# nguyenduchuyiu/marl-delivery

Hardware: AMD Instinct MI355X
Metric: agent-steps/sec (whole node), map1 5-agent 4096 envs, 1/2/4/8 MI355X (higher is better)
Workload: dtype int32+fp64

## Files before the change

### marl-delivery_amd/csrc/mdl_step_halves.hpp

```cpp
#pragma once

constexpr int HALF = 32;
constexpr int HALF_NC = 4;
constexpr int HALVES_MAX_P = HALF * HALF_NC;
constexpr int HALF_CAND = 136;

__device__ __forceinline__ uint32_t half_min_u32(uint32_t m) {
    m = row_min_u32(m);
    const auto r = __builtin_amdgcn_permlane16_swap(m, m, false, false);
    return r[0] < r[1] ? r[0] : r[1];
}

constexpr size_t HALF_GREC = (size_t)HALF_NC * 64 * 8, HALF_GPS = (size_t)HALF_NC * 64 * 2;
__host__ __device__ constexpr size_t halves_scratch_bytes() {
    return HALF_GREC + HALF_GPS + 64 * (size_t)HALF_NC + 2 * (size_t)HALF_CAND * 8;
}

struct HalvesLayout {
    static constexpr int G = HALF, NC = HALF_NC;
    static constexpr uint32_t ROFF_MASK = 0x1fu;
    static constexpr uint32_t RESET_OFF_MASK = 0xffu;
    static constexpr size_t FLAG_OFF = HALF_GREC + HALF_GPS;
    static constexpr bool RANK_BEFORE_RESET = false;
    __device__ static __forceinline__ bool stores_robot(const GroupLane q) { return (q.lane & 16) == 0; }

    struct Near {
        int stc[NC];
        uint64_t anyw;
        uint64_t* cand;
        int nwg;
    };
    template <bool STALE>
    __device__ static __forceinline__ void near_pre(Near& nr, const GroupLane q, unsigned char* slice,
                                                    const uint32_t (&ps0)[NC], const uint64_t (&td)[NC], int t0, bool, int) {
        uint64_t wvm[NC];
        bool wv[NC];
        nr.anyw = 0;
#pragma unroll
        for (int c = 0; c < NC; c++) {
            wv[c] = !(MDL_ABLATE & 64) && trk_waiting<STALE>(ps0[c], td[c], t0);
            nr.stc[c] = pk_start(td[c]);
            wvm[c] = ballot(wv[c]);
            nr.anyw |= wvm[c];
        }
        nr.cand = (uint64_t*)(slice + HALF_GREC + HALF_GPS + 64 * NC) + q.g * HALF_CAND;
        nr.nwg = 0;
        if (nr.anyw) {
            int n0 = 0, n1 = 0;
#pragma unroll
            for (int c = 0; c < NC; c++) {
                const int lo = popc64(wvm[c] & 0x00000000ffffffffull);
                const int below = (int)__builtin_amdgcn_mbcnt_hi((uint32_t)(wvm[c] >> 32),
                                                                 __builtin_amdgcn_mbcnt_lo((uint32_t)wvm[c], 0u));
                const int idx = below + (q.g ? n1 - lo : n0);
                const uint32_t j = (uint32_t)(c * HALF + q.gl);
                const uint32_t klo = (near_order<STALE, HALF * NC>(ps0[c], j) << 7) | j;
                if (wv[c]) nr.cand[idx] = (uint64_t)(uint32_t)nr.stc[c] | ((uint64_t)klo << 32);
                n0 += lo;
                n1 += popc64(wvm[c] & 0xffffffff00000000ull);
            }
            const int nh = q.g ? n1 : n0;
            nr.nwg = (max(n0, n1) + 3) & ~3;
            for (int k = nh + q.gl; k < nr.nwg; k += HALF) nr.cand[k] = 0x0000ffffffffffffull;
        }
    }
    __device__ static __forceinline__ void near_post(const Near& nr, const GroupLane q, bool, bool act, int pcell, int cell,
                                                     uint32_t& Midle, uint32_t& Mcan, int& best_cell) {
        if (nr.anyw && !(MDL_ABLATE & 32)) {
            const uint64_t* cp = nr.cand + ((q.lane >> 4) & 1);
            uint32_t kmin = 0xffffffffu;
            uint64_t hmc = 0;
            for (int i0 = 0; i0 < nr.nwg; i0 += 4) {
                const uint64_t ce = cp[i0], cf = cp[i0 + 2];
                const uint32_t ke = __builtin_amdgcn_sad_hi_u8((uint32_t)pcell, (uint32_t)ce, (uint32_t)(ce >> 32));
                const uint32_t kf = __builtin_amdgcn_sad_hi_u8((uint32_t)pcell, (uint32_t)cf, (uint32_t)(cf >> 32));
                kmin = min(kmin, min(ke, kf));
                hmc |= ballot((int)(uint32_t)ce == cell) | ballot((int)(uint32_t)cf == cell);
            }
            {
                const auto r = __builtin_amdgcn_permlane16_swap(kmin, kmin, false, false);
                kmin = r[0] < r[1] ? r[0] : r[1];
            }
            const uint32_t h16 = (uint32_t)(((hmc >> q.gbase) | (hmc >> (q.gbase + 16))) & 0xffffull);
            Mcan = ((h16 >> q.ri) & 1u) ? ~0u : 0u;
            const int js = (int)(kmin & 127u);
            const int sl = (q.gbase + (js & 31)) << 2;
            int bc = __builtin_amdgcn_ds_bpermute(sl, nr.stc[0]);
#pragma unroll
            for (int c = 1; c < NC; c++) {
                const int v = __builtin_amdgcn_ds_bpermute(sl, nr.stc[c]);
                bc = (js >> 5) == c ? v : bc;
            }
            const bool found = act && kmin < (509u << 16);
            Midle = lmask(found && (kmin >> 16) <= 3u);
            best_cell = found ? bc : -1;
        }
    }

    __device__ static __forceinline__ void gather_put(unsigned char* slice, int lane, const uint32_t (&ps0)[NC],
                                                      const uint64_t (&pk)[NC], const uint64_t (&td)[NC]) {
        uint64_t* grec = (uint64_t*)slice;
        uint16_t* gps = (uint16_t*)(slice + HALF_GREC);
#pragma unroll
        for (int c = 0; c < NC; c++) {
            grec[c * 64 + lane] = (uint64_t)tgt_dl(pk[c]) | ((uint64_t)tgt_dl(td[c]) << 32);
            gps[c * 64 + lane] = (uint16_t)ps0[c];
        }
    }
    __device__ static __forceinline__ void gather_get(unsigned char* slice, const GroupLane q, int pj, uint32_t& g_pf,
                                                      uint32_t& g_pk, uint32_t& g_td) {
        const int gi = ((pj >> 5) & (NC - 1)) * 64 + q.gbase + (pj & 31);
        const uint64_t gv = ((const uint64_t*)slice)[gi];
        g_pf = ((const uint16_t*)(slice + HALF_GREC))[gi], g_pk = (uint32_t)gv, g_td = (uint32_t)(gv >> 32);
    }

    __device__ static __forceinline__ void partners(const GroupLane q, bool act, bool mover, uint64_t, int prop, int cell,
                                                    bool& blocked, int& occ) {
        const uint32_t wd = (mover ? (uint32_t)prop : 0xffffu) | ((act ? (uint32_t)cell : 0xfffeu) << 16);
        const int g8 = (q.lane & 16) >> 1;
        uint32_t hk = 0;
        int ok = -1;
#pragma unroll
        for (int k = 0; k < 8; k++) {
            const uint32_t wj = (uint32_t)__builtin_amdgcn_ds_bpermute((q.gbase + g8 + k) << 2, (int)wd);
            hk |= (wj & 0xffffu) == (uint32_t)prop ? (1u << k) : 0u;
            ok = (wj >> 16) == (uint32_t)prop ? k : ok;
        }
        uint32_t hit = hk << g8;
        occ = ok < 0 ? -1 : ok + g8;
        {
            const auto rh = __builtin_amdgcn_permlane16_swap(hit, hit, false, false);
            hit = rh[0] | rh[1];
            const auto ro = __builtin_amdgcn_permlane16_swap((uint32_t)occ, (uint32_t)occ, false, false);
            occ = max((int)ro[0], (int)ro[1]);
        }
        blocked = (hit & ((1u << q.ri) - 1u)) != 0u;
    }

    __device__ static __forceinline__ void pickups(const GroupLane q, unsigned char* slice, uint32_t nw, bool picker,
                                                   uint64_t pickers, const int (&sw)[NC], int cell, int& cnew) {
        constexpr uint32_t NONE = 255u;
        if (nw & NW_SMALLMAP) {
            uint32_t* pb = (uint32_t*)slice + q.g * 128;
            auto word_of = [](int cl) { return (((uint32_t)cl >> 7) | (((uint32_t)cl >> 5) & 1u)) & 127u; };
            wave_sync();
            reinterpret_cast<u32x4*>((uint32_t*)slice)[q.lane] = u32x4{0u, 0u, 0u, 0u};
            wave_sync();
            if (picker && stores_robot(q)) atomicOr(&pb[word_of(cell)], 1u << (cell & 31));
            wave_sync();
            uint64_t left = pickers & 0x0000ffff0000ffffull;
#pragma unroll
            for (int c = 0; c < NC; c++) {
                const uint32_t bit = __builtin_amdgcn_ubfe(pb[word_of(sw[c])], (uint32_t)sw[c] & 31u, 1u);
                const uint64_t mt = ballot((sw[c] >= 0) & (bit != 0u));
                for (uint64_t m = mt; m && left; m &= m - 1) {
                    const int j = ffs64(m);
                    const uint64_t who = ballot(cell == rdl(sw[c], j)) & left & (0xffffull << (j & 32));
                    if (who) {
                        const int i = ffs64(who);
                        left &= ~(1ull << i);
                        cnew = (q.lane & ~16) == i ? c * HALF + (j & 31) + 1 : cnew;
                    }
                }
            }
        } else
        for (uint32_t u = rows_union(pickers); u; u &= u - 1) {
            const int J = __ffs((int)u) - 1;
            const int ci = __builtin_amdgcn_ds_bpermute((q.rbase + J) << 2, cell);
            uint32_t k = NONE;
#pragma unroll
            for (int c = NC - 1; c >= 0; c--) k = sw[c] == ci ? (uint32_t)(c * HALF + q.gl) : k;
            k = half_min_u32(k);
            cnew = (q.ri == J && picker && k != NONE) ? (int)k + 1 : cnew;
        }
    }

    __device__ static __forceinline__ float agent_sum(float s_lane, int) {
        const float r8 = s_lane + dppf<0x128>(s_lane);
        const float s2 = r8 + dppf<0xB1>(r8);
        const float c4 = s2 + dppf<0x4E>(s2);
        const float d = c4 + dppf<0x124>(c4);
        return 0.0f + row_bcastf<0>(d);
    }

    __device__ static __forceinline__ ResetLds reset_robots(uint32_t (&)[NC], unsigned char* slice, const GroupLane q,
                                                            const DevParams& p, int P, uint32_t, int er2, int gb, int mi,
                                                            int mvoff, bool store, GLOBAL uint32_t* robe) {
        ResetLds L = reset_carve(slice, P);
        const int mr = rdl(mi, gb);
        const MapDesc md = p.maps[mr];
        const int nc = do_reset(p, er2, md, L, false);
        const int ncr = __builtin_amdgcn_ds_bpermute(q.ri << 2, nc);
        if (store) *robe = rob_pack(ncr, 0, p.movevalid_cell[(uint32_t)(mvoff + ncr)]);
        return L;
    }
};
```

### marl-delivery_amd/csrc/mdl_step_multi.hpp

```cpp
#pragma once

struct GroupLane {
    int lane;
    int g, gl, gbase;
    int rbase, ri;
};
template <bool STALE, int MAXP>
__device__ __forceinline__ uint32_t near_order(uint32_t f, uint32_t j) {
    return STALE ? ((f & PS_SURVIVOR) ? (f >> PS_RANK_SHIFT) : (uint32_t)MAXP + j) : j;
}

#include "mdl_step_rows.hpp"
#include "mdl_step_halves.hpp"

template <bool STALE, int G, int NC>
__device__ __forceinline__ void rank_survivors(uint32_t (&ps)[NC], const GroupLane q, int P, int gb, bool mine) {
    constexpr uint64_t GMASK = ~0ull >> (64 - G);
    uint32_t rk[NC], tq[NC];
#pragma unroll
    for (int c = 0; c < NC; c++) {
        rk[c] = 0;
        tq[c] = order_key<STALE>(ps[c], c * G + q.gl);
    }
#pragma unroll
    for (int c2 = 0; c2 < NC; c2++) {
        uint64_t pm = ballot(c2 * G + q.gl < P && (ps[c2] & PS_PRESENT)) & (GMASK << gb);
        while (pm) {
            const uint32_t ki = (uint32_t)rdl((int)tq[c2], ffs64(pm));
            pm &= pm - 1;
#pragma unroll
            for (int c = 0; c < NC; c++) rk[c] += ki < tq[c] ? 1u : 0u;
        }
    }
#pragma unroll
    for (int c = 0; c < NC; c++) {
        if (mine) {
            if (c * G + q.gl < P && (ps[c] & PS_PRESENT)) {
                ps[c] = (ps[c] & PS_FLAGS) | PS_SURVIVOR | (rk[c] << PS_RANK_SHIFT);
            } else {
                ps[c] &= PS_STATUS;
            }
        }
    }
}

template <class L, bool STALE, int NFULL>
__device__ __forceinline__ void step_groups(const uint32_t* __restrict__ rob_pre, const uint64_t* __restrict__ pkg_pre,
                                            const uint16_t* __restrict__ pst_pre, const u32x4* __restrict__ es_pre,
                                            const uint64_t* __restrict__ trk_pre, const uint8_t* __restrict__ act_pre,
                                            uint32_t ap, uint32_t nw, const StepArgs& args) {
    constexpr int G = L::G, LG = G == 16 ? 4 : 5, NC = L::NC, NG = WAVE / G, MAX_P = G * NC;
    static_assert(G == 1 << LG, "groups of 16 or 32 lanes");
    constexpr uint64_t GMASK = ~0ull >> (64 - G);
    static_assert(NC == 4, "one flag byte per package slot, a lane's NC slots in one 32-bit load");
    constexpr int MAX_OFF = (NG - 1) * MAX_P + (G - 1) + (NC - 1) * G;
    static_assert(MAX_OFF < PKG_PAD && MAX_OFF <= 0xff, "step_groups: package loads stay inside the buffers' padding");
    extern __shared__ __align__(16) unsigned char smem[];
    const DevParams& p = args.p;
    const StepPre pre(rob_pre, pkg_pre, pst_pre, es_pre, trk_pre, act_pre, ap, nw);
    const int A = pre.A, P = pre.P;

    const int wave = wave_id();
    const int lane = lane_id();
    const int w = pre.slot() * pre.wpb + wave;
    const int e0 = NG * w;
    if (wave >= pre.wpb || e0 >= pre.n) return;
    const GroupLane q{lane, lane >> LG, lane & (G - 1), lane & (WAVE - G), lane & 48, lane & 15};
    const bool live = e0 + q.g < pre.n;
    const int ge = live ? q.g : 0;
    const bool act = live && q.ri < A;
    const bool rstore = L::stores_robot(q);

    const uint32_t roff = (uint32_t)(q.g * A + q.ri);
    const uint32_t roff_c = (act ? roff : 0u) & L::ROFF_MASK;
    const uint32_t rv_ld = (pre.rob + (size_t)e0 * A)[roff_c];
    const uint32_t ar_ld = (pre.act + (size_t)e0 * A)[roff_c];
    uint64_t pk[NC], td[NC];
    uint32_t ps[NC], ps_in[NC];
    bool dirty[NC];
    GLOBAL const uint64_t* pkge = pre.pkg + (size_t)e0 * P;
    GLOBAL const uint16_t* pste = pre.pst + (size_t)e0 * P;
    GLOBAL const uint64_t* trke = pre.trk + (size_t)e0 * P;
    bool pv[NC];
    const uint32_t lb = (uint32_t)(ge * P + q.gl) & 0xffu;
#pragma unroll
    for (int c = 0; c < NC; c++) {
        pv[c] = c < NFULL || c * G + q.gl < P;
        pk[c] = pkge[lb + c * G];
        ps[c] = pste[lb + c * G];
        td[c] = STALE ? trke[lb + c * G] : 0ull;
        dirty[c] = false;
    }
    const uint32_t erow = (uint32_t)ge & (NG - 1);
    const uint32_t t_ld = ((GLOBAL const uint32_t*)(pre.es + e0))[4u * erow];
    const uint64_t tot_ld = ((GLOBAL const uint64_t*)(pre.es + e0))[2u * erow + 1u];
    KargPtr kap = (KargPtr)((__attribute__((address_space(4))) const char*)__builtin_amdgcn_kernarg_segment_ptr() +
                            offsetof(StepKarg, args));
    const double cst = kap->p.cost_fold[q.gl];
    __builtin_amdgcn_sched_barrier(0);
    const uint32_t rv = act ? rv_ld : 0u;
    int araw = act ? (int)(ar_ld & 0xffu) : 0;
    const uint32_t t_rec = t_ld;
    const uint64_t tot_rec = tot_ld;
#pragma unroll
    for (int c = 0; c < NC; c++) {
        if (c >= NFULL) {
            pk[c] = pv[c] ? pk[c] : ~0ull;
            ps[c] = pv[c] ? ps[c] : (uint32_t)ST_DELIVERED;
            td[c] = pv[c] ? td[c] : ~0ull;
        }
        ps_in[c] = ps[c];
    }
    const int fmt = args.fmt, auto_reset = args.auto_reset, lds_stride = args.lds_stride;
    const int T = p.T;
    unsigned char* slice = smem + (size_t)wave * lds_stride;
    int mvoff = p.maps[0].mvc_off;
    int mi = 0;
    if (nw & NW_MAP) {
        mi = (int)((GLOBAL const uint8_t*)p.env_map)[e0 + ge];
#pragma unroll
        for (int k = 1; k < MAX_MAPS; k++) mvoff = (mi == k) ? p.maps[k].mvc_off : mvoff;
    }
    int cell = rob_cell(rv), carry = rob_carry(rv);
    uint32_t vmask = rob_valid(rv);
    const int t0 = (int)t_rec;
    const double tot_cur = __hiloint2double((int)(uint32_t)(tot_rec >> 32), (int)(uint32_t)tot_rec);

    int mv, op;
    decode_action(araw, fmt, mv, op);
    mv = act ? mv : MV_S;
    op = act ? op : 0;
    uint32_t ps0[NC];
#pragma unroll
    for (int c = 0; c < NC; c++) {
        ps0[c] = ps[c];
        if (!STALE || !(ps0[c] & PS_SURVIVOR)) td[c] = pk[c];
    }

    typename L::Near nr;
    L::template near_pre<STALE>(nr, q, slice, ps0, td, t0, act, cell);

    const int pj = carry - 1;
    unsigned char* flb = slice + L::FLAG_OFF;
    L::gather_put(slice, lane, ps0, pk, td);
    ((uint32_t*)flb)[lane] = 0;
    wave_sync();
    uint32_t g_pf, g_pk, g_td;
    L::gather_get(slice, q, pj, g_pf, g_pk, g_td);

    const int pcell = cell, pcarry = carry;
    const int prop = move_proposal(act, cell, vmask, mv);
    const bool mover = !(MDL_ABLATE & 4) && act && prop != cell;
    const uint64_t movers = ballot(mover);
    const uint32_t pvm = (uint32_t)(p.movevalid_cell + mvoff)[(uint32_t)prop];
    uint64_t moved = 0;
    if (movers) {
        bool blocked;
        int occ;
        L::partners(q, act, mover, movers, prop, cell, blocked, occ);
        const uint32_t Mbase = lmask(mover && !blocked), Mfree = lmask(occ < 0);
        moved = ballot((Mbase & Mfree) != 0u);
        if (ballot((Mbase & ~Mfree) != 0u)) {
            const int oln = q.rbase + (occ & 15);
            for (int it = 0; it < A; it++) {
                const uint64_t nm = ballot((Mbase & (Mfree | vbit(moved, oln))) != 0u);
                if (nm == moved) break;
                moved = nm;
            }
        }
        if ((moved >> lane) & 1ull) cell = prop;
    }
    const int n_cost = (int)__popc(row_bits(moved, q.rbase));

    const bool picker = !(MDL_ABLATE & 8) && act && op == 1 && carry == 0;
    const uint64_t pickers = ballot(picker);
    int cnew = carry;
    if (pickers) {
        int sw[NC];
#pragma unroll
        for (int c = 0; c < NC; c++) sw[c] = (ps[c] & PS_STATUS) == ST_WAITING ? pk_start(pk[c]) : -2;
        L::pickups(q, slice, nw, picker, pickers, sw, cell, cnew);
    }
    const bool picked = cnew != carry;
    carry = cnew;
    const int g_tgt = (int)(g_pk & 0xffffu), g_dl = (int)(g_pk >> 16);
    const bool drop = act && op == 2 && carry != 0 && g_tgt == cell;
    const uint64_t dmask = ballot(drop), omask = ballot(drop && t0 <= g_dl);
    constexpr uint32_t F_CHG = 8u, F_CARRY = 4u;
    {
        const int fs = drop ? pj : carry - 1;
        const uint32_t fv = picked ? (F_CHG | F_CARRY | (uint32_t)ST_IN_TRANSIT)
                            : drop ? (F_CHG | (uint32_t)ST_DELIVERED) : F_CARRY;
        if (act && rstore && carry != 0) flb[(q.gbase + (fs & (G - 1))) * NC + (fs >> LG)] = (unsigned char)fv;
    }
    carry = drop ? 0 : carry;
    wave_sync();
    const uint32_t fw = ((const uint32_t*)flb)[lane];
#pragma unroll
    for (int c = 0; c < NC; c++) {
        const uint32_t f = fw >> (8 * c);
        const uint32_t clr = (0u - ((f >> 3) & 1u)) & PS_STATUS;
        ps[c] = (ps[c] & ~clr) | (f & PS_STATUS);
    }
    double rr;
    {
        const int src = (q.gbase + n_cost) << 2;
        const uint32_t lo = (uint32_t)__builtin_amdgcn_ds_bpermute(src, (int)__double2loint(cst));
        const uint32_t hi = (uint32_t)__builtin_amdgcn_ds_bpermute(src, (int)__double2hiint(cst));
        rr = __hiloint2double((int)hi, (int)lo);
    }
    const uint32_t drow = row_bits(dmask, q.rbase), orow = row_bits(omask, q.rbase);
    if (dmask) {
        double DR = p.delivery_reward, DL = p.delay_reward;
        pin(DR);
        pin(DL);
        for (uint32_t u = rows_union(dmask); u; u &= u - 1) {
            const int i = __ffs((int)u) - 1;
            const double add = ((orow >> i) & 1u) ? DR : DL;
            rr = ((drow >> i) & 1u) ? rr + add : rr;
        }
    }
    const uint32_t rfl = (n_cost ? RT_MOVE : 0u) | (orow ? RT_ONTIME : 0u) | ((drow & ~orow) ? RT_LATE : 0u);
    const int t1 = t0 + 1;
    const double total = tot_cur + rr;

    uint32_t undel = 0;
    uint64_t spawned = 0;
#pragma unroll
    for (int c = 0; c < NC; c++) {
        undel |= (ps[c] & PS_STATUS) ^ (uint32_t)ST_DELIVERED;
        const bool sp = pk_st(pk[c]) == t1;
        spawned |= ballot(sp);
        ps[c] = sp ? ((ps[c] & ~PS_STATUS) | ST_WAITING) : ps[c];
    }
    const uint32_t alldel = lmask(((ballot(undel != 0u) >> q.gbase) & GMASK) == 0ull);
    const bool done = (lmask(live) & (lmask(t1 == T) | alldel)) != 0u;

    float s_lane;
    {
        const ShapeMasks<STALE> M(act, pcarry, carry, P, g_pf, pcell, cell, mv, op);
        uint32_t Midle = 0, Mcan = 0;
        int best_cell = -1;
        L::near_post(nr, q, M.need_can(), act, pcell, cell, Midle, Mcan, best_cell);
        const ShapeConsts C(p);
        s_lane = shape_terms<STALE>(M, C, (int)(g_td & 0xffffu), (int)(g_td >> 16), t1, best_cell, Midle, Mcan, pcell, cell);
    }
    const float shaped = (float)rr + L::agent_sum(s_lane, A);

    const bool do_rst = done && auto_reset;
    const uint64_t rst = ballot(do_rst);
    if (STALE && !(MDL_ABLATE & 2) && (ballot(picked) | dmask | spawned)) {
#pragma unroll
        for (int c = 0; c < NC; c++) {
            const bool ins = !do_rst && (pk_st(pk[c]) == t1) && !(ps[c] & PS_PRESENT);
            ps[c] = ins ? ((ps[c] & PS_STATUS) | PS_PRESENT) : ps[c];
            td[c] = ins ? pk[c] : td[c];
            dirty[c] = dirty[c] || ins;
            const uint32_t m_p = lmask((ps[c] & PS_PRESENT) != 0u && !do_rst);
            const uint32_t m_c = lmask(((fw >> (8 * c)) & F_CARRY) != 0u);
            const uint32_t m_t = lmask((ps[c] & PS_TRANSIT) != 0u);
            ps[c] = (ps[c] | (PS_TRANSIT & m_c & m_p)) & (PS_STATUS | ~(m_p & ~m_c & m_t));
        }
    }

    const int t_out = do_rst ? 0 : t1;
    const double total_out = do_rst ? 0.0 : total;
    vmask = (((moved >> lane) & 1ull) && !do_rst) ? pvm : vmask;
    asm volatile("" : "+v"(vmask));
    GLOBAL double* rop = (GLOBAL double*)kap->r_out;
    GLOBAL float* shp = (GLOBAL float*)kap->sh_out;
    GLOBAL uint8_t* dnp = (GLOBAL uint8_t*)kap->done_out;
    GLOBAL uint32_t* robw = (GLOBAL uint32_t*)kap->p.rob;
    GLOBAL uint16_t* pstw = (GLOBAL uint16_t*)kap->p.pstate;
    GLOBAL uint64_t* trkw = (GLOBAL uint64_t*)kap->p.trk;
    GLOBAL u32x4* esw = (GLOBAL u32x4*)kap->p.es;
    const uint32_t er = (uint32_t)q.g & (NG - 1);
    if (live && q.gl == 0) {
        if (rop) (rop + e0)[er] = rr;
        if (shp) (shp + e0)[er] = shaped;
        if (dnp) (dnp + e0)[er] = done ? 1 : 0;
        (esw + e0)[er] = u32x4{(uint32_t)t_out, rfl, (uint32_t)__double2loint(total_out),
                               (uint32_t)__double2hiint(total_out)};
    }
    if (live && q.gl == 0 && done) {
        ((GLOBAL double*)p.ep_total + e0)[er] = total;
        ((GLOBAL int32_t*)p.ep_len + e0)[er] = t1;
    }
    if (act && rstore && !do_rst) (robw + (size_t)e0 * A)[roff] = rob_pack(cell, carry, vmask);
    const size_t eb = (size_t)e0 * P;
#pragma unroll
    for (int c = 0; c < NC; c++) {
        const uint32_t o = lb + c * G;
        if (live && pv[c] && !do_rst && ps[c] != ps_in[c]) (pstw + eb)[o] = (uint16_t)ps[c];
        if (STALE && live && pv[c] && dirty[c]) (trkw + eb)[o] = td[c];
    }

    if (rst) {
        GLOBAL uint64_t* pkgw = (GLOBAL uint64_t*)kap->p.pkg;
        wave_sync();
        constexpr uint64_t FIRST = ~0ull / GMASK;
        for (uint64_t m = rst & FIRST; m; m &= m - 1) {
            const int gb = ffs64(m);
            const int er2 = e0 + (gb >> LG);
            const bool mine = q.gbase == gb;
            if (STALE && L::RANK_BEFORE_RESET) rank_survivors<STALE, G, NC>(ps, q, P, gb, mine);
            ResetLds R = L::reset_robots(ps, slice, q, p, P, nw, er2, gb, mi, mvoff, mine && act && rstore,
                                         robw + (size_t)e0 * A + roff);
            if (STALE && !L::RANK_BEFORE_RESET) rank_survivors<STALE, G, NC>(ps, q, P, gb, mine);
#pragma unroll
            for (int c = 0; c < NC; c++) {
                const int j = c * G + q.gl;
                if (mine && j < P) {
                    const uint64_t npk = R.pk[j];
                    uint32_t nps = (uint32_t)R.pst[j] | (STALE ? (ps[c] & ~PS_STATUS) : 0u);
                    const uint32_t o = (uint32_t)(q.g * P + j) & L::RESET_OFF_MASK;
                    if (STALE) {
                        const bool ins = (pk_st(npk) == 0) & !(nps & PS_PRESENT);
                        nps = ins ? ((nps & PS_STATUS) | PS_PRESENT) : nps;
                        if (ins) (trkw + eb)[o] = npk;
                        const uint32_t upd = (nps & PS_TRANSIT) ? (nps & PS_STATUS) : nps;
                        nps = (nps & PS_PRESENT) ? upd : nps;
                    }
                    (pkgw + eb)[o] = npk;
                    (pstw + eb)[o] = (uint16_t)nps;
                }
            }
            wave_sync();
        }
    }
}

template <bool STALE, int AU, int NC, int NFULL>
__global__ __launch_bounds__(256) void k_step_rows(const uint32_t* __restrict__ rob_pre,
                                                   const uint64_t* __restrict__ pkg_pre,
                                                   const uint16_t* __restrict__ pst_pre,
                                                   const u32x4* __restrict__ es_pre,
                                                   const uint64_t* __restrict__ trk_pre,
                                                   const uint8_t* __restrict__ act_pre, uint32_t ap, uint32_t nw,
                                                   StepArgs args) {
    step_groups<RowsLayout<AU, NC>, STALE, NFULL>(rob_pre, pkg_pre, pst_pre, es_pre, trk_pre, act_pre, ap, nw, args);
}

template <bool STALE, int NFULL>
__global__ __launch_bounds__(256) void k_step_halves(const uint32_t* __restrict__ rob_pre,
                                                     const uint64_t* __restrict__ pkg_pre,
                                                     const uint16_t* __restrict__ pst_pre,
                                                     const u32x4* __restrict__ es_pre,
                                                     const uint64_t* __restrict__ trk_pre,
                                                     const uint8_t* __restrict__ act_pre, uint32_t ap, uint32_t nw,
                                                     StepArgs args) {
    step_groups<HalvesLayout, STALE, NFULL>(rob_pre, pkg_pre, pst_pre, es_pre, trk_pre, act_pre, ap, nw, args);
}
```

### marl-delivery_amd/csrc/mdl_step_rows.hpp

```cpp
#pragma once

constexpr int ROW = 16;
constexpr int ROWS_MAX_P = ROW * 4;

template <int J>
__device__ __forceinline__ int row_bcast(int v) {
    return __builtin_amdgcn_update_dpp(0, v, 0x150 + J, 0xf, 0xf, false);
}
template <int J>
__device__ __forceinline__ float row_bcastf(float v) {
    return __int_as_float(row_bcast<J>(__float_as_int(v)));
}
__device__ __forceinline__ uint32_t row_bits(uint64_t m, int rbase) { return (uint32_t)(m >> rbase) & 0xffffu; }
__device__ __forceinline__ uint32_t rows_union(uint64_t m) { return (uint32_t)((m | (m >> 16) | (m >> 32) | (m >> 48)) & 0xffffull); }
__device__ __forceinline__ uint32_t row_min_u32(uint32_t m) {
    const int id = (int)0xffffffff;
    uint32_t t;
    t = (uint32_t)__builtin_amdgcn_update_dpp(id, (int)m, 0xB1, 0xf, 0xf, false); m = t < m ? t : m;
    t = (uint32_t)__builtin_amdgcn_update_dpp(id, (int)m, 0x4E, 0xf, 0xf, false); m = t < m ? t : m;
    t = (uint32_t)__builtin_amdgcn_update_dpp(id, (int)m, 0x124, 0xf, 0xf, false); m = t < m ? t : m;
    t = (uint32_t)__builtin_amdgcn_update_dpp(id, (int)m, 0x128, 0xf, 0xf, false); m = t < m ? t : m;
    return m;
}
__device__ __forceinline__ uint32_t row_or_u32(uint32_t m) {
    m |= (uint32_t)__builtin_amdgcn_update_dpp(0, (int)m, 0xB1, 0xf, 0xf, false);
    m |= (uint32_t)__builtin_amdgcn_update_dpp(0, (int)m, 0x4E, 0xf, 0xf, false);
    m |= (uint32_t)__builtin_amdgcn_update_dpp(0, (int)m, 0x124, 0xf, 0xf, false);
    m |= (uint32_t)__builtin_amdgcn_update_dpp(0, (int)m, 0x128, 0xf, 0xf, false);
    return m;
}

template <int AU>
__device__ __forceinline__ float row_np_sum(float v, int A) {
    static_assert(AU >= 1 && AU <= 8, "row_np_sum: AU <= 8");
    constexpr int L = AU < 8 ? AU : 7;
    if (AU == 8 && A == 8) {
        const float a = v + dppf<0xB1>(v);
        const float b = a + dppf<0x4E>(a);
        const float c = b + dppf<0x124>(b);
        return 0.0f + row_bcastf<4>(c);
    }
    float t = v;
#pragma unroll
    for (int i = 1; i < L; i++) t = v + dppf<0x111>(t);
    return row_bcastf<L - 1>(t);
}

__device__ __forceinline__ uint32_t tgt_dl(uint64_t v) {
    return __builtin_amdgcn_perm((uint32_t)(v >> 32), (uint32_t)v, 0x07060302u);
}

__host__ __device__ constexpr size_t rows_scratch_bytes(int NC) { return (size_t)NC * 64 * 16 + 64 * (size_t)NC; }
constexpr size_t ROWS_PS_STASH = rows_scratch_bytes(4) - 4 * 64 * 2;
static_assert(reset_lds_bytes(ROWS_MAX_P) <= ROWS_PS_STASH, "k_step_rows: the reset scratch ends before the stashed state words");

template <int AU, int NC_>
struct RowsLayout {
    static_assert(AU >= 1 && AU <= 8, "k_step_rows: A <= 8");
    static_assert(NC_ == 4, "k_step_rows: P <= 64 (the only form built and tested)");
    static constexpr int G = ROW, NC = NC_;
    static constexpr uint32_t ROFF_MASK = 0x3fu;
    static constexpr uint32_t RESET_OFF_MASK = 0x1ffu;
    static constexpr size_t FLAG_OFF = (size_t)NC * 64 * 16;
    static constexpr bool RANK_BEFORE_RESET = true;
    __device__ static __forceinline__ bool stores_robot(const GroupLane) { return true; }

    struct Near {
        int swv[NC];
        uint64_t anyw;
        uint32_t Midle;
        int best_cell;
    };
    template <bool STALE>
    __device__ static __forceinline__ void near_pre(Near& nr, const GroupLane q, unsigned char*, const uint32_t (&ps0)[NC],
                                                    const uint64_t (&td)[NC], int t0, bool act, int cell) {
        int stc[NC];
        uint32_t klo[NC];
        nr.anyw = 0;
#pragma unroll
        for (int c = 0; c < NC; c++) {
            const bool wv = !(MDL_ABLATE & 64) && trk_waiting<STALE>(ps0[c], td[c], t0);
            stc[c] = pk_start(td[c]);
            nr.swv[c] = wv ? stc[c] : -1;
            const uint32_t j = (uint32_t)(c * ROW + q.gl);
            klo[c] = wv ? (near_order<STALE, ROW * NC>(ps0[c], j) << 7) | j : 0xffffu;
            nr.anyw |= ballot(wv);
        }
        nr.Midle = 0;
        nr.best_cell = -1;
        if (nr.anyw && !(MDL_ABLATE & 32)) {
            uint32_t kmin = 0xffffffffu;
#define MDL_NEAR(J)                                                                                  \
    if constexpr (J < AU) {                                                                          \
        const int pa = row_bcast<J>(cell);                                                           \
        uint32_t k = 0xffffffffu;                                                                    \
        _Pragma("unroll") for (int c = 0; c < NC; c++) {                                             \
            const uint32_t kc = __builtin_amdgcn_sad_hi_u8((uint32_t)pa, (uint32_t)nr.swv[c], klo[c]); \
            k = kc < k ? kc : k;                                                                     \
        }                                                                                            \
        k = row_min_u32(k);                                                                          \
        kmin = q.gl == J ? k : kmin;                                                                 \
    }
            MDL_NEAR(0) MDL_NEAR(1) MDL_NEAR(2) MDL_NEAR(3) MDL_NEAR(4) MDL_NEAR(5) MDL_NEAR(6) MDL_NEAR(7)
#undef MDL_NEAR
            const int js = (int)(kmin & 127u);
            const int sl = (q.gbase + (js & 15)) << 2;
            int bc = __builtin_amdgcn_ds_bpermute(sl, stc[0]);
#pragma unroll
            for (int c = 1; c < NC; c++) {
                const int v = __builtin_amdgcn_ds_bpermute(sl, stc[c]);
                bc = (js >> 4) == c ? v : bc;
            }
            const bool found = act && kmin < (509u << 16);
            nr.Midle = lmask(found && (kmin >> 16) <= 3u);
            nr.best_cell = found ? bc : -1;
        }
    }
    __device__ static __forceinline__ void near_post(const Near& nr, const GroupLane q, bool need_can, bool, int, int cell,
                                                     uint32_t& Midle, uint32_t& Mcan, int& best_cell) {
        Midle = nr.Midle;
        best_cell = nr.best_cell;
        if (nr.anyw && !(MDL_ABLATE & 32)) {
            if (ballot(need_can)) {
                uint32_t hm = 0;
#define MDL_CAN(J)                                                                                   \
    if constexpr (J < AU) {                                                                          \
        const int ca = row_bcast<J>(cell);                                                           \
        bool h = false;                                                                              \
        _Pragma("unroll") for (int c = 0; c < NC; c++) h = h | (nr.swv[c] == ca);                    \
        hm |= h ? (1u << J) : 0u;                                                                    \
    }
                MDL_CAN(0) MDL_CAN(1) MDL_CAN(2) MDL_CAN(3) MDL_CAN(4) MDL_CAN(5) MDL_CAN(6) MDL_CAN(7)
#undef MDL_CAN
                hm = row_or_u32(hm);
                Mcan = ((hm >> q.gl) & 1u) ? ~0u : 0u;
            }
        }
    }

    __device__ static __forceinline__ void gather_put(unsigned char* slice, int lane, const uint32_t (&ps0)[NC],
                                                      const uint64_t (&pk)[NC], const uint64_t (&td)[NC]) {
        u32x4* grec = (u32x4*)slice;
#pragma unroll
        for (int c = 0; c < NC; c++) grec[c * 64 + lane] = u32x4{ps0[c], tgt_dl(pk[c]), tgt_dl(td[c]), 0u};
    }
    __device__ static __forceinline__ void gather_get(unsigned char* slice, const GroupLane q, int pj, uint32_t& g_pf,
                                                      uint32_t& g_pk, uint32_t& g_td) {
        const u32x4 g = ((const u32x4*)slice)[((pj >> 4) & (NC - 1)) * 64 + q.gbase + (pj & 15)];
        g_pf = g.x, g_pk = g.y, g_td = g.z;
    }

    __device__ static __forceinline__ void partners(const GroupLane q, bool act, bool, uint64_t movers, int prop, int cell,
                                                    bool& blocked, int& occ) {
        const int propx = act ? prop : -2, cellx = act ? cell : -3;
        int pjs[AU], cjs[AU];
#define MDL_ROWB(J)                          \
    if constexpr (J < AU) {                  \
        pjs[J] = row_bcast<J>(propx);        \
        cjs[J] = row_bcast<J>(cellx);        \
    }
        MDL_ROWB(0) MDL_ROWB(1) MDL_ROWB(2) MDL_ROWB(3) MDL_ROWB(4) MDL_ROWB(5) MDL_ROWB(6) MDL_ROWB(7)
#undef MDL_ROWB
        uint32_t hit = 0;
        occ = -1;
#pragma unroll
        for (int j = 0; j < AU; j++) {
            hit |= pjs[j] == prop ? (1u << j) : 0u;
            occ = cjs[j] == prop ? j : occ;
        }
        blocked = (hit & ((1u << q.gl) - 1u) & row_bits(movers, q.gbase)) != 0u;
    }

    __device__ static __forceinline__ void pickups(const GroupLane q, unsigned char*, uint32_t, bool picker,
                                                   uint64_t pickers, const int (&sw)[NC], int cell, int& cnew) {
        constexpr uint32_t NONE = 255u;
        const uint32_t pu = rows_union(pickers);
#define MDL_PICK(J)                                                                                  \
    if constexpr (J < AU) {                                                                          \
        if (pu & (1u << J)) {                                                                        \
            const int ci = row_bcast<J>(cell);                                                       \
            uint32_t k = NONE;                                                                       \
            _Pragma("unroll") for (int c = NC - 1; c >= 0; c--) k = sw[c] == ci ? (uint32_t)(c * ROW + q.gl) : k; \
            k = row_min_u32(k);                                                                      \
            cnew = (q.gl == J && picker && k != NONE) ? (int)k + 1 : cnew;                           \
        }                                                                                            \
    }
        MDL_PICK(0) MDL_PICK(1) MDL_PICK(2) MDL_PICK(3) MDL_PICK(4) MDL_PICK(5) MDL_PICK(6) MDL_PICK(7)
#undef MDL_PICK
    }

    __device__ static __forceinline__ float agent_sum(float s_lane, int A) { return row_np_sum<AU>(s_lane, A); }

    __device__ static __forceinline__ ResetLds reset_robots(uint32_t (&ps)[NC], unsigned char* slice, const GroupLane q,
                                                            const DevParams& p, int P, uint32_t nw, int er2, int, int, int,
                                                            bool store, GLOBAL uint32_t* robe) {
        uint16_t* pss = (uint16_t*)(slice + ROWS_PS_STASH);
#pragma unroll
        for (int c = 0; c < NC; c++) pss[c * 64 + q.lane] = (uint16_t)ps[c];
        ResetLds L = reset_carve(slice, P);
        const int mr = (nw & NW_MAP) ? (int)((GLOBAL const uint8_t*)p.env_map)[er2] : 0;
        const MapDesc md = p.maps[mr];
        const int nc = do_reset(p, er2, md, L, false);
        const int ncr = __builtin_amdgcn_ds_bpermute(q.ri << 2, nc);
        if (store) *robe = rob_pack(ncr, 0, p.movevalid_cell[(uint32_t)(md.mvc_off + ncr)]);
#pragma unroll
        for (int c = 0; c < NC; c++) ps[c] = pss[c * 64 + q.lane];
        return L;
    }
};
```

Baseline: 4.946 billion.

## Defer nearest-package search and skip it for agents that don't need it

```diff
diff --git a/marl-delivery_amd/csrc/mdl_step_halves.hpp b/marl-delivery_amd/csrc/mdl_step_halves.hpp
--- a/marl-delivery_amd/csrc/mdl_step_halves.hpp
+++ b/marl-delivery_amd/csrc/mdl_step_halves.hpp
@@ -64,6 +64,9 @@
             for (int k = nh + q.gl; k < nr.nwg; k += HALF) nr.cand[k] = 0x0000ffffffffffffull;
         }
     }
+    template <bool STALE>
+    __device__ static __forceinline__ void near_search(Near&, const GroupLane, const uint32_t (&)[NC], const uint64_t (&)[NC],
+                                                       bool, bool, int) {}
     __device__ static __forceinline__ void near_post(const Near& nr, const GroupLane q, bool, bool act, int pcell, int cell,
                                                      uint32_t& Midle, uint32_t& Mcan, int& best_cell) {
         if (nr.anyw && !(MDL_ABLATE & 32)) {
diff --git a/marl-delivery_amd/csrc/mdl_step_multi.hpp b/marl-delivery_amd/csrc/mdl_step_multi.hpp
--- a/marl-delivery_amd/csrc/mdl_step_multi.hpp
+++ b/marl-delivery_amd/csrc/mdl_step_multi.hpp
@@ -8,6 +8,11 @@
 template <bool STALE, int MAXP>
 __device__ __forceinline__ uint32_t near_order(uint32_t f, uint32_t j) {
     return STALE ? ((f & PS_SURVIVOR) ? (f >> PS_RANK_SHIFT) : (uint32_t)MAXP + j) : j;
+}
+
+template <bool STALE>
+__device__ __forceinline__ bool trk_has(uint32_t f) {
+    return STALE ? (f & PS_PRESENT) != 0u : ((f & PS_STATUS) == ST_WAITING || (f & PS_STATUS) == ST_IN_TRANSIT);
 }
 
 #include "mdl_step_rows.hpp"
@@ -172,6 +177,9 @@
     }
     const int n_cost = (int)__popc(row_bits(moved, q.rbase));
 
+    L::template near_search<STALE>(nr, q, ps0, td, act && !(pcarry != 0 && pcarry <= P && trk_has<STALE>(g_pf)), act,
+                                   pcell);
+
     const bool picker = !(MDL_ABLATE & 8) && act && op == 1 && carry == 0;
     const uint64_t pickers = ballot(picker);
     int cnew = carry;
@@ -186,22 +194,28 @@
     const int g_tgt = (int)(g_pk & 0xffffu), g_dl = (int)(g_pk >> 16);
     const bool drop = act && op == 2 && carry != 0 && g_tgt == cell;
     const uint64_t dmask = ballot(drop), omask = ballot(drop && t0 <= g_dl);
+    const int t1 = t0 + 1;
+    uint64_t spawned = 0;
+#pragma unroll
+    for (int c = 0; c < NC; c++) spawned |= ballot(pk_st(pk[c]) == t1);
+    const uint64_t ev = ballot(picked) | dmask | spawned;
     constexpr uint32_t F_CHG = 8u, F_CARRY = 4u;
-    {
+    uint32_t fw = 0;
+    if (STALE ? ev : (ballot(picked) | dmask)) {
         const int fs = drop ? pj : carry - 1;
         const uint32_t fv = picked ? (F_CHG | F_CARRY | (uint32_t)ST_IN_TRANSIT)
                             : drop ? (F_CHG | (uint32_t)ST_DELIVERED) : F_CARRY;
         if (act && rstore && carry != 0) flb[(q.gbase + (fs & (G - 1))) * NC + (fs >> LG)] = (unsigned char)fv;
+        wave_sync();
+        fw = ((const uint32_t*)flb)[lane];
+#pragma unroll
+        for (int c = 0; c < NC; c++) {
+            const uint32_t f = fw >> (8 * c);
+            const uint32_t clr = (0u - ((f >> 3) & 1u)) & PS_STATUS;
+            ps[c] = (ps[c] & ~clr) | (f & PS_STATUS);
+        }
     }
     carry = drop ? 0 : carry;
-    wave_sync();
-    const uint32_t fw = ((const uint32_t*)flb)[lane];
-#pragma unroll
-    for (int c = 0; c < NC; c++) {
-        const uint32_t f = fw >> (8 * c);
-        const uint32_t clr = (0u - ((f >> 3) & 1u)) & PS_STATUS;
-        ps[c] = (ps[c] & ~clr) | (f & PS_STATUS);
-    }
     double rr;
     {
         const int src = (q.gbase + n_cost) << 2;
@@ -221,16 +235,13 @@
         }
     }
     const uint32_t rfl = (n_cost ? RT_MOVE : 0u) | (orow ? RT_ONTIME : 0u) | ((drow & ~orow) ? RT_LATE : 0u);
-    const int t1 = t0 + 1;
     const double total = tot_cur + rr;
 
     uint32_t undel = 0;
-    uint64_t spawned = 0;
 #pragma unroll
     for (int c = 0; c < NC; c++) {
         undel |= (ps[c] & PS_STATUS) ^ (uint32_t)ST_DELIVERED;
         const bool sp = pk_st(pk[c]) == t1;
-        spawned |= ballot(sp);
         ps[c] = sp ? ((ps[c] & ~PS_STATUS) | ST_WAITING) : ps[c];
     }
     const uint32_t alldel = lmask(((ballot(undel != 0u) >> q.gbase) & GMASK) == 0ull);
@@ -249,7 +260,7 @@
 
     const bool do_rst = done && auto_reset;
     const uint64_t rst = ballot(do_rst);
-    if (STALE && !(MDL_ABLATE & 2) && (ballot(picked) | dmask | spawned)) {
+    if (STALE && !(MDL_ABLATE & 2) && ev) {
 #pragma unroll
         for (int c = 0; c < NC; c++) {
             const bool ins = !do_rst && (pk_st(pk[c]) == t1) && !(ps[c] & PS_PRESENT);
diff --git a/marl-delivery_amd/csrc/mdl_step_rows.hpp b/marl-delivery_amd/csrc/mdl_step_rows.hpp
--- a/marl-delivery_amd/csrc/mdl_step_rows.hpp
+++ b/marl-delivery_amd/csrc/mdl_step_rows.hpp
@@ -73,33 +73,43 @@
     };
     template <bool STALE>
     __device__ static __forceinline__ void near_pre(Near& nr, const GroupLane q, unsigned char*, const uint32_t (&ps0)[NC],
-                                                    const uint64_t (&td)[NC], int t0, bool act, int cell) {
-        int stc[NC];
-        uint32_t klo[NC];
+                                                    const uint64_t (&td)[NC], int t0, bool, int) {
         nr.anyw = 0;
 #pragma unroll
         for (int c = 0; c < NC; c++) {
             const bool wv = !(MDL_ABLATE & 64) && trk_waiting<STALE>(ps0[c], td[c], t0);
-            stc[c] = pk_start(td[c]);
-            nr.swv[c] = wv ? stc[c] : -1;
-            const uint32_t j = (uint32_t)(c * ROW + q.gl);
-            klo[c] = wv ? (near_order<STALE, ROW * NC>(ps0[c], j) << 7) | j : 0xffffu;
+            nr.swv[c] = wv ? pk_start(td[c]) : -1;
             nr.anyw |= ballot(wv);
         }
         nr.Midle = 0;
         nr.best_cell = -1;
-        if (nr.anyw && !(MDL_ABLATE & 32)) {
+    }
+    template <bool STALE>
+    __device__ static __forceinline__ void near_search(Near& nr, const GroupLane q, const uint32_t (&ps0)[NC],
+                                                       const uint64_t (&td)[NC], bool need, bool act, int cell) {
+        const uint32_t nu = rows_union(ballot(need));
+        if (nr.anyw && nu && !(MDL_ABLATE & 32)) {
+            int stc[NC];
+            uint32_t klo[NC];
+#pragma unroll
+            for (int c = 0; c < NC; c++) {
+                stc[c] = pk_start(td[c]);
+                const uint32_t j = (uint32_t)(c * ROW + q.gl);
+                klo[c] = nr.swv[c] >= 0 ? (near_order<STALE, ROW * NC>(ps0[c], j) << 7) | j : 0xffffu;
+            }
             uint32_t kmin = 0xffffffffu;
 #define MDL_NEAR(J)                                                                                  \
     if constexpr (J < AU) {                                                                          \
-        const int pa = row_bcast<J>(cell);                                                           \
-        uint32_t k = 0xffffffffu;                                                                    \
-        _Pragma("unroll") for (int c = 0; c < NC; c++) {                                             \
-            const uint32_t kc = __builtin_amdgcn_sad_hi_u8((uint32_t)pa, (uint32_t)nr.swv[c], klo[c]); \
-            k = kc < k ? kc : k;                                                                     \
+        if (nu & (1u << J)) {                                                                        \
+            const int pa = row_bcast<J>(cell);                                                       \
+            uint32_t k = 0xffffffffu;                                                                \
+            _Pragma("unroll") for (int c = 0; c < NC; c++) {                                         \
+                const uint32_t kc = __builtin_amdgcn_sad_hi_u8((uint32_t)pa, (uint32_t)nr.swv[c], klo[c]); \
+                k = kc < k ? kc : k;                                                                 \
+            }                                                                                        \
+            k = row_min_u32(k);                                                                      \
+            kmin = q.gl == J ? k : kmin;                                                             \
         }                                                                                            \
-        k = row_min_u32(k);                                                                          \
-        kmin = q.gl == J ? k : kmin;                                                                 \
     }
             MDL_NEAR(0) MDL_NEAR(1) MDL_NEAR(2) MDL_NEAR(3) MDL_NEAR(4) MDL_NEAR(5) MDL_NEAR(6) MDL_NEAR(7)
 #undef MDL_NEAR
@@ -121,14 +131,17 @@
         Midle = nr.Midle;
         best_cell = nr.best_cell;
         if (nr.anyw && !(MDL_ABLATE & 32)) {
-            if (ballot(need_can)) {
+            const uint32_t cu = rows_union(ballot(need_can));
+            if (cu) {
                 uint32_t hm = 0;
 #define MDL_CAN(J)                                                                                   \
     if constexpr (J < AU) {                                                                          \
-        const int ca = row_bcast<J>(cell);                                                           \
-        bool h = false;                                                                              \
-        _Pragma("unroll") for (int c = 0; c < NC; c++) h = h | (nr.swv[c] == ca);                    \
-        hm |= h ? (1u << J) : 0u;                                                                    \
+        if (cu & (1u << J)) {                                                                        \
+            const int ca = row_bcast<J>(cell);                                                       \
+            bool h = false;                                                                          \
+            _Pragma("unroll") for (int c = 0; c < NC; c++) h = h | (nr.swv[c] == ca);                \
+            hm |= h ? (1u << J) : 0u;                                                                \
+        }                                                                                            \
     }
                 MDL_CAN(0) MDL_CAN(1) MDL_CAN(2) MDL_CAN(3) MDL_CAN(4) MDL_CAN(5) MDL_CAN(6) MDL_CAN(7)
 #undef MDL_CAN
```

After: 4.952 billion (median of 3 runs). Within noise of the previous version (+0.1%).
